# iPieter/llmq

Measured on AMD Instinct MI355X. Metric: output_tokens_per_sec (Tower-Plus-9B continuous-batching serving decode), higher is better.
Workload: dtype bf16; 1 GPU; model=tower-plus-9b (gemma-2-9b arch, random init), global_batch=512, seq_len=1024, parallelism=dp1, kv_cache_dtype=auto

## Files before the change

### llmq_amd/engine/model_runner.py

```python

from __future__ import annotations

import logging
import time
from typing import Dict, List, Optional, Tuple

import numpy as np
import torch

from llmq_amd import ops
from llmq_amd.engine.config import EngineConfig
from llmq_amd.engine.forward_meta import ChunkGather, DecodeMeta, MixedMeta, PrefillMeta
from llmq_amd.engine.kv_cache import KVCache
from llmq_amd.engine.models.llama import CausalLM
from llmq_amd.engine.scheduler import ScheduledBatch, Sequence

logger = logging.getLogger(__name__)


def _buckets(max_bs: int) -> List[int]:
    sizes = [1, 2, 4, 8, 16, 24, 32, 48, 64, 96, 128, 192, 256, 384, 512]
    out = [b for b in sizes if b < max_bs]
    out.append(max_bs)
    return out
# ... 4 lines not shown
        self,
        model: CausalLM,
        kv_cache: KVCache,
        config: EngineConfig,
        device: torch.device,
        max_model_len: int,
    ):
        self.model = model
        self.kv_cache = kv_cache
        self.config = config
        self.device = device
        self.max_model_len = max_model_len
        self.block_size = kv_cache.block_size
        self.max_blocks_per_seq = (max_model_len + self.block_size - 1) // self.block_size
        self.use_graphs = (
            config.enable_hipgraph
            and not config.enforce_eager
            and device.type == "cuda"
        )
        self._graphs: Dict[int, torch.cuda.CUDAGraph] = {}
        self._graph_pool = None
        self.sampling_generator = torch.Generator(device=device if device.type == "cuda" else "cpu")
        self.sampling_generator.manual_seed(config.seed)
        self._sample_step = 0
        self._sample_bufs: Dict[str, Dict[str, torch.Tensor]] = {}
        if self.use_graphs:
            self._alloc_static_buffers()


    def _alloc_static_buffers(self) -> None:
        B = min(self.config.max_num_seqs, self.config.hipgraph_max_batch)
        dev = self.device
        self.graph_max_bs = B
        self.in_ids = torch.zeros(B, dtype=torch.long, device=dev)
        self.in_pos = torch.zeros(B, dtype=torch.long, device=dev)
        self.in_slots = torch.zeros(B, dtype=torch.long, device=dev)
        self.in_block_tables = torch.zeros(
            B, self.max_blocks_per_seq, dtype=torch.int32, device=dev
        )
        self.in_context_lens = torch.ones(B, dtype=torch.int32, device=dev)
        self.out_hidden = torch.zeros(
            B, self.model.spec.hidden_size, dtype=self.model.dtype, device=dev
        )
        self.h_ids = torch.zeros(B, dtype=torch.long, pin_memory=True)
        self.h_pos = torch.zeros(B, dtype=torch.long, pin_memory=True)
        self.h_slots = torch.zeros(B, dtype=torch.long, pin_memory=True)
        self.h_block_tables = torch.zeros(
            B, self.max_blocks_per_seq, dtype=torch.int32, pin_memory=True
        )
        self.h_context_lens = torch.ones(B, dtype=torch.int32, pin_memory=True)
        self._staged_rows: List[Tuple[int, int, int]] = [(-1, -1, 0)] * B

    def capture_graphs(self) -> None:
        if not self.use_graphs:
            return
        t0 = time.perf_counter()
        torch.cuda.synchronize()
        for bs in reversed(_buckets(self.graph_max_bs)):
            meta = DecodeMeta(
                block_tables=self.in_block_tables[:bs],
                context_lens=self.in_context_lens[:bs],
                slot_mapping=self.in_slots[:bs],
            )
            out = self.model.forward(self.in_ids[:bs], self.in_pos[:bs], self.kv_cache, meta)
            torch.cuda.synchronize()
            graph = torch.cuda.CUDAGraph()
            with torch.cuda.graph(graph, pool=self._graph_pool):
                out = self.model.forward(
                    self.in_ids[:bs], self.in_pos[:bs], self.kv_cache, meta
                )
                self.out_hidden[:bs].copy_(out)
            if self._graph_pool is None:
                self._graph_pool = graph.pool()
            self._graphs[bs] = graph
        torch.cuda.synchronize()
        logger.info(
            "captured %d decode hipGraphs (max_bs=%d) in %.1fs",
            len(self._graphs), self.graph_max_bs, time.perf_counter() - t0,
        )

    def _bucket_for(self, bs: int) -> Optional[int]:
        for b in _buckets(self.graph_max_bs):
            if b >= bs:
                return b
        return None


    def _build_prefill_meta(self, pseqs, chunks, dev) -> tuple:
        bs = self.block_size
        ids: List[int] = []
        pos: List[int] = []
        slots: List[int] = []
        cu = [0]
        cu_k = [0]
        rel_last: List[int] = []
        any_chunk = any(start > 0 for (start, _e) in chunks)
        g_blocks: List[int] = []
        g_offs: List[int] = []
        past_dst: List[int] = []
        fresh_dst: List[int] = []
        krow = 0
        for seq, (start, end) in zip(pseqs, chunks):
            n = end - start
            ids.extend(seq.token_ids[start:end])
            pos.extend(range(start, end))
            bt = seq.block_table
            slots.extend(bt[p // bs] * bs + (p % bs) for p in range(start, end))
            if end == seq.num_tokens:
                rel_last.append(cu[-1] + n - 1)
            cu.append(cu[-1] + n)
            if any_chunk:
                for p in range(start):
                    g_blocks.append(bt[p // bs])
                    g_offs.append(p % bs)
                    past_dst.append(krow)
                    krow += 1
                for i in range(cu[-2], cu[-1]):
                    fresh_dst.append(krow)
                    krow += 1
            cu_k.append(cu_k[-1] + end)
        slot_mapping = torch.tensor(slots, dtype=torch.long, device=dev)
        gather = None
        if any_chunk:
            gather = ChunkGather(
                cu_seqlens_k=torch.tensor(cu_k, dtype=torch.int32, device=dev),
                blocks=torch.tensor(g_blocks, dtype=torch.long, device=dev),
                offs=torch.tensor(g_offs, dtype=torch.long, device=dev),
                past_dst=torch.tensor(past_dst, dtype=torch.long, device=dev),
                fresh_dst=torch.tensor(fresh_dst, dtype=torch.long, device=dev),
                total_k=krow,
            )
        meta = PrefillMeta(
            cu_seqlens=torch.tensor(cu, dtype=torch.int32, device=dev),
            max_seqlen=max(e - st for (st, e) in chunks),
            slot_mapping=slot_mapping,
            gather=gather,
        )
        return ids, pos, slot_mapping, meta, rel_last

    @torch.no_grad()
    def execute_prefill(self, seqs: List[Sequence], chunks=None, buf_name: str = "main") -> torch.Tensor:
        if chunks is None:
            chunks = [(0, s.num_tokens) for s in seqs]
        dev = self.device
        ids, pos, slot_mapping, meta, rel_last = self._build_prefill_meta(
            seqs, chunks, dev
        )
        input_ids = torch.tensor(ids, dtype=torch.long, device=dev)
        positions = torch.tensor(pos, dtype=torch.long, device=dev)
        hidden = self.model.forward(input_ids, positions, self.kv_cache, meta)
        if not rel_last:
            return torch.empty(0, dtype=torch.long, device=dev)
        last_hidden = hidden[torch.tensor(rel_last, dtype=torch.long, device=dev)]
        logits = self.model.compute_logits(last_hidden)
        sample_seqs = [s for s, (st, e) in zip(seqs, chunks) if e == s.num_tokens]
        return self._sample(logits, sample_seqs, buf_name)


    @torch.no_grad()
    def execute_mixed(self, batch: "ScheduledBatch") -> torch.Tensor:
        dev = self.device
        dseqs = batch.seqs[: batch.n_decode]
        pseqs = batch.seqs[batch.n_decode :]
        chunks = batch.chunks or [(0, s.num_tokens) for s in pseqs]
        bs = self.block_size
        nd = len(dseqs)

        ids = [s.token_ids[-1] for s in dseqs]
        pos = [s.num_tokens - 1 for s in dseqs]
        slots = [s.block_table[p // bs] * bs + (p % bs) for s, p in zip(dseqs, pos)]
        ctx = [s.num_tokens for s in dseqs]
        p_ids, p_pos, p_slots, pmeta, rel_last = self._build_prefill_meta(
            pseqs, chunks, dev
        )
        ids.extend(p_ids)
        pos.extend(p_pos)

        block_tables = torch.zeros(
            nd, max(len(s.block_table) for s in dseqs), dtype=torch.int32, device=dev
        )
        bt_np = np.zeros(tuple(block_tables.shape), dtype=np.int32)
        for i, s in enumerate(dseqs):
            bt_np[i, : len(s.block_table)] = s.block_table
        block_tables.copy_(torch.from_numpy(bt_np))
        d_slots = torch.tensor(slots, dtype=torch.long, device=dev)
        slot_mapping = torch.cat([d_slots, p_slots])
        meta = MixedMeta(
            n_decode=nd,
            decode=DecodeMeta(
                block_tables=block_tables,
                context_lens=torch.tensor(ctx, dtype=torch.int32, device=dev),
                slot_mapping=d_slots,
            ),
            prefill=pmeta,
            slot_mapping=slot_mapping,
        )
        input_ids = torch.tensor(ids, dtype=torch.long, device=dev)
        positions = torch.tensor(pos, dtype=torch.long, device=dev)
        hidden = self.model.forward(input_ids, positions, self.kv_cache, meta)
        last_idx = list(range(nd)) + [nd + r for r in rel_last]
        last_hidden = hidden[torch.tensor(last_idx, dtype=torch.long, device=dev)]
        logits = self.model.compute_logits(last_hidden)
        sample_seqs = list(dseqs) + [
            s for s, (st, e) in zip(pseqs, chunks) if e == s.num_tokens
        ]
        return self._sample(logits, sample_seqs)


    @torch.no_grad()
    def execute_decode(self, seqs: List[Sequence], force_eager: bool = False) -> torch.Tensor:
        dev = self.device
        B = len(seqs)
        bs = self.block_size
        ids = [s.token_ids[-1] for s in seqs]
        pos = [s.num_tokens - 1 for s in seqs]
        slots = [s.block_table[p // bs] * bs + (p % bs) for s, p in zip(seqs, pos)]
        ctx = [s.num_tokens for s in seqs]

        bucket = self._bucket_for(B) if (self.use_graphs and not force_eager) else None
        if bucket is not None and bucket in self._graphs:
            return self._decode_with_graph(seqs, bucket, ids, pos, slots, ctx)

        block_tables = torch.zeros(
            B, max(len(s.block_table) for s in seqs), dtype=torch.int32, device=dev
        )
        bt_np = np.zeros(tuple(block_tables.shape), dtype=np.int32)
        for i, s in enumerate(seqs):
            bt_np[i, : len(s.block_table)] = s.block_table
        block_tables.copy_(torch.from_numpy(bt_np))
        meta = DecodeMeta(
            block_tables=block_tables,
            context_lens=torch.tensor(ctx, dtype=torch.int32, device=dev),
            slot_mapping=torch.tensor(slots, dtype=torch.long, device=dev),
        )
        input_ids = torch.tensor(ids, dtype=torch.long, device=dev)
        positions = torch.tensor(pos, dtype=torch.long, device=dev)
        hidden = self.model.forward(input_ids, positions, self.kv_cache, meta)
        logits = self.model.compute_logits(hidden)
        return self._sample(logits, seqs)

    def _decode_with_graph(
        self, seqs: List[Sequence], bucket: int, ids, pos, slots, ctx
    ) -> torch.Tensor:
        B = len(seqs)
        self.h_ids[:B] = torch.tensor(ids, dtype=torch.long)
        self.h_pos[:B] = torch.tensor(pos, dtype=torch.long)
        self.h_slots[:B] = torch.tensor(slots, dtype=torch.long)
        self.h_context_lens[:B] = torch.tensor(ctx, dtype=torch.int32)
        self.h_context_lens[B:bucket] = 1
        bt_np = self.h_block_tables.numpy()
        max_w = 1
        for i, s in enumerate(seqs):
            n = len(s.block_table)
            if n > max_w:
                max_w = n
            if self._staged_rows[i] != (s.uid, s.num_preemptions, n):
                bt_np[i, :n] = s.block_table
                self._staged_rows[i] = (s.uid, s.num_preemptions, n)
        if B < bucket:
            self.h_slots[B:bucket] = 0
            self.h_ids[B:bucket] = 0
            self.h_pos[B:bucket] = 0
            for i in range(B, bucket):
                if self._staged_rows[i] != (-1, -1, 0):
                    bt_np[i, :1] = 0
                    self._staged_rows[i] = (-1, -1, 0)
        self.in_ids[:bucket].copy_(self.h_ids[:bucket], non_blocking=True)
        self.in_pos[:bucket].copy_(self.h_pos[:bucket], non_blocking=True)
        self.in_slots[:bucket].copy_(self.h_slots[:bucket], non_blocking=True)
        self.in_context_lens[:bucket].copy_(self.h_context_lens[:bucket], non_blocking=True)
        self.in_block_tables[:bucket, :max_w].copy_(
            self.h_block_tables[:bucket, :max_w], non_blocking=True
        )
        self._graphs[bucket].replay()
        logits = self.model.compute_logits(self.out_hidden[:B])
        return self._sample(logits, seqs)


    def _sample_buf(self, name: str, B: int, dev) -> Dict[str, torch.Tensor]:
        buf = self._sample_bufs.get(name)
        if buf is None or buf["out"].numel() < B:
            cap = max(B, self.config.max_num_seqs)
            buf = {
                "out": torch.empty(cap, dtype=torch.int64, device=dev),
                "keys": torch.empty(cap, dtype=torch.int64, device=dev),
                "temps": torch.empty(cap, dtype=torch.float32, device=dev),
                "temps_h": torch.empty(cap, dtype=torch.float32, pin_memory=True),
                "seeds": torch.empty(cap, dtype=torch.int32, device=dev),
                "seeds_h": torch.empty(cap, dtype=torch.int32, pin_memory=True),
                "pos": torch.empty(cap, dtype=torch.int32, device=dev),
                "pos_h": torch.empty(cap, dtype=torch.int32, pin_memory=True),
            }
            self._sample_bufs[name] = buf
        return buf

    def _sample(self, logits: torch.Tensor, seqs: List[Sequence],
                buf_name: str = "main") -> torch.Tensor:
        dev = logits.device
        self._sample_step += 1
        simple = all(
            s.params.top_k == 0 and s.params.top_p >= 1.0 for s in seqs
        )
        if dev.type == "cuda":
            B = len(seqs)
            buf = self._sample_buf(buf_name, B, dev)
            th = buf["temps_h"]
            sh = buf["seeds_h"]
            ph = buf["pos_h"]
            for i, s in enumerate(seqs):
                th[i] = s.params.temperature
                rs = s.params.seed
                if rs is None:
                    sh[i] = 0
                else:
                    v = rs & 0x7FFFFFFF
                    sh[i] = v if v else 0x1E3779B9
                ph[i] = s.output_len
            buf["temps"][:B].copy_(th[:B], non_blocking=True)
            buf["seeds"][:B].copy_(sh[:B], non_blocking=True)
            buf["pos"][:B].copy_(ph[:B], non_blocking=True)
            logits_f = logits.float()
            bounds = None
            if not simple:
                tps = torch.tensor([s.params.top_p for s in seqs],
                                   dtype=torch.float32, device=dev)
                tks = torch.tensor([s.params.top_k for s in seqs],
                                   dtype=torch.int64, device=dev)
                bounds = ops.topk_topp_bound(
                    logits_f, buf["temps"][:B], tps, tks)
            ops.sample_gumbel_argmax(
                buf["out"][:B], buf["keys"][:B], logits_f,
                buf["temps"][:B], buf["seeds"][:B],
                buf["pos"][:B], self.config.seed, self._sample_step, bounds,
            )
            return buf["out"][:B]
        temps = torch.tensor([s.params.temperature for s in seqs], dtype=torch.float32, device=dev)
        tps = torch.tensor([s.params.top_p for s in seqs], dtype=torch.float32, device=dev)
        tks = torch.tensor([s.params.top_k for s in seqs], dtype=torch.int64, device=dev)
        out = ops.sample_tokens(logits, temps, tps, tks, self.sampling_generator)
        seeded = [
            i for i, s in enumerate(seqs)
            if s.params.seed is not None and s.params.temperature > 0
        ]
        if seeded:
            idx = torch.tensor(seeded, dtype=torch.long, device=dev)
            rows = logits[idx].float().cpu()
            temps_c, tps_c, tks_c = temps[idx].cpu(), tps[idx].cpu(), tks[idx].cpu()
            redraw = torch.empty(len(seeded), dtype=out.dtype)
            for j, i in enumerate(seeded):
                s = seqs[i]
                g = torch.Generator(device="cpu")
                g.manual_seed((s.params.seed << 20) ^ s.output_len)
                redraw[j] = ops.sample_tokens(
                    rows[j : j + 1], temps_c[j : j + 1], tps_c[j : j + 1],
                    tks_c[j : j + 1], g,
                )[0]
            out[idx] = redraw.to(out.device)
        return out
```

### llmq_amd/engine/models/llama.py

```python

from __future__ import annotations

import math
import os
from typing import Dict, List, Optional, Union

import torch
import torch.nn.functional as F

from llmq_amd import ops
from llmq_amd.engine.forward_meta import DecodeMeta, MixedMeta, PrefillMeta
from llmq_amd.engine.kv_cache import KVCache
from llmq_amd.engine.model_specs import ModelSpec
from llmq_amd.parallel import get_tp_group


_USE_SKINNY_GEMM = os.environ.get("LLMQ_SKINNY_GEMM", "0") not in ("0", "false", "")


def _proj(x: torch.Tensor, w: torch.Tensor, bias=None) -> torch.Tensor:
    if (_USE_SKINNY_GEMM and x.is_cuda and x.dtype == torch.bfloat16
            and x.shape[0] <= 1024 and w.shape[1] % 64 == 0
            and w.shape[0] % 4 == 0):
        return ops.skinny_gemm(x, w, bias)
# ... 104 lines not shown
        h = self.spec.hidden_size
        std = 0.02
        out_std = std / math.sqrt(2 * self.spec.num_layers)
        fill(self.embedding, std)
        for lw in self.layers:
            lw.input_norm.fill_(1.0 - self.norm_offset)
            fill(lw.qkv, std)
            if lw.qkv_bias is not None:
                lw.qkv_bias.zero_()
            fill(lw.o, out_std)
            lw.pre_mlp_norm.fill_(1.0 - self.norm_offset)
            fill(lw.gate_up, std)
            fill(lw.down, out_std)
            if lw.post_attn_norm is not None:
                lw.post_attn_norm.fill_(1.0 - self.norm_offset)
                lw.post_mlp_norm.fill_(1.0 - self.norm_offset)
        self.final_norm.fill_(1.0 - self.norm_offset)
        if not self.spec.tied_embeddings:
            fill(self.lm_head, std)

    def named_tensors(self) -> Dict[str, torch.Tensor]:
        out = {"embedding": self.embedding, "final_norm": self.final_norm}
        if not self.spec.tied_embeddings:
            out["lm_head"] = self.lm_head
        for i, lw in enumerate(self.layers):
            p = f"layers.{i}."
            out[p + "input_norm"] = lw.input_norm
            out[p + "qkv"] = lw.qkv
            if lw.qkv_bias is not None:
                out[p + "qkv_bias"] = lw.qkv_bias
            out[p + "o"] = lw.o
            out[p + "pre_mlp_norm"] = lw.pre_mlp_norm
            out[p + "gate_up"] = lw.gate_up
            out[p + "down"] = lw.down
            if lw.post_attn_norm is not None:
                out[p + "post_attn_norm"] = lw.post_attn_norm
                out[p + "post_mlp_norm"] = lw.post_mlp_norm
        return out

    def weight_bytes(self) -> int:
        return sum(t.numel() * t.element_size() for t in self.named_tensors().values())


    def _norm(self, x: torch.Tensor, w: torch.Tensor) -> torch.Tensor:
        return ops.rmsnorm(x, w, self.spec.rms_eps, self.norm_offset)

    def _prefill_attn(self, q, k, v, pmeta, kv_cache, layer: int, window: int):
        s = self.spec
        g = pmeta.gather
        if g is None:
            return ops.varlen_prefill_attention(
                q, k, v, pmeta.cu_seqlens, pmeta.max_seqlen, s.scale,
                s.attn_softcap, window,
            )
        KVH, D = k.shape[1], k.shape[2]
        k_att = q.new_empty(g.total_k, KVH, D)
        v_att = q.new_empty(g.total_k, KVH, D)
        past_k = kv_cache.k[layer][g.blocks, :, g.offs].to(q.dtype)
        past_v = kv_cache.v[layer][g.blocks, :, g.offs].to(q.dtype)
        k_att.index_copy_(0, g.past_dst, past_k)
        v_att.index_copy_(0, g.past_dst, past_v)
        k_att.index_copy_(0, g.fresh_dst, k)
        v_att.index_copy_(0, g.fresh_dst, v)
        return ops.varlen_prefill_attention(
            q, k_att, v_att, pmeta.cu_seqlens, pmeta.max_seqlen, s.scale,
            s.attn_softcap, window, cu_seqlens_k=g.cu_seqlens_k,
        )

    @torch.no_grad()
    def forward(
        self,
        input_ids: torch.Tensor,
        positions: torch.Tensor,
        kv_cache: KVCache,
        meta: Union[PrefillMeta, DecodeMeta, MixedMeta],
    ) -> torch.Tensor:
        s = self.spec
        tp = get_tp_group() if self.tp_size > 1 else None
        x = F.embedding(input_ids, self.embedding)
        if s.embedding_scale:
            x = x * math.sqrt(s.hidden_size)
            x = x.to(self.dtype)
        residual = x
        h = self._norm(x, self.layers[0].input_norm)
        n_layers = len(self.layers)
        for i, lw in enumerate(self.layers):
            qkv = _proj(h, lw.qkv, lw.qkv_bias)
            q, k, v = qkv.split([self.q_size, self.kv_size, self.kv_size], dim=-1)
            T = q.shape[0]
            q = q.view(T, self.heads, s.head_dim)
            k = k.view(T, self.kv_heads, s.head_dim)
            v = v.view(T, self.kv_heads, s.head_dim)
            ops.rope_and_cache(
                q, k, v, kv_cache.k[i], kv_cache.v[i], positions,
                self.rope_cache, meta.slot_mapping,
            )
            window = s.sliding_window if s.layer_uses_sliding_window(i) else 0
            if meta.is_prefill:
                attn = self._prefill_attn(q, k, v, meta, kv_cache, i, window)
            elif meta.is_mixed:
                nd = meta.n_decode
                attn_d = ops.paged_decode_attention(
                    q[:nd], kv_cache.k[i], kv_cache.v[i],
                    meta.decode.block_tables, meta.decode.context_lens,
                    s.scale, s.attn_softcap, window,
                )
                attn_p = self._prefill_attn(
                    q[nd:], k[nd:], v[nd:], meta.prefill, kv_cache, i, window
                )
                attn = torch.cat([attn_d, attn_p], dim=0)
            else:
                attn = ops.paged_decode_attention(
                    q, kv_cache.k[i], kv_cache.v[i], meta.block_tables,
                    meta.context_lens, s.scale, s.attn_softcap, window,
                )
            attn_out = _proj(attn.reshape(T, self.q_size), lw.o)
            if tp is not None:
                attn_out = tp.all_reduce(attn_out)
            if s.post_norms:
                h, residual = ops.norm_add_norm(
                    attn_out, residual, lw.post_attn_norm, lw.pre_mlp_norm,
                    s.rms_eps, self.norm_offset,
                )
            else:
                h, residual = ops.fused_add_rmsnorm(
                    attn_out, residual, lw.pre_mlp_norm, s.rms_eps, self.norm_offset
                )
            gate_up = _proj(h, lw.gate_up)
            act = ops.gelu_tanh_and_mul(gate_up) if s.gelu else ops.silu_and_mul(gate_up)
            mlp_out = _proj(act, lw.down)
            if tp is not None:
                mlp_out = tp.all_reduce(mlp_out)
            w_next = (
                self.layers[i + 1].input_norm if i + 1 < n_layers else self.final_norm
            )
            if s.post_norms:
                h, residual = ops.norm_add_norm(
                    mlp_out, residual, lw.post_mlp_norm, w_next,
                    s.rms_eps, self.norm_offset,
                )
            else:
                h, residual = ops.fused_add_rmsnorm(
                    mlp_out, residual, w_next, s.rms_eps, self.norm_offset
                )
        return h

    @torch.no_grad()
    def compute_logits(self, hidden: torch.Tensor) -> torch.Tensor:
        logits = _proj(hidden, self.lm_head).float()
        cap = self.spec.final_softcap
        if cap and cap > 0:
            logits = torch.tanh(logits / cap) * cap
        return logits
```

### llmq_amd/ops/__init__.py

```python

from __future__ import annotations

import os
from pathlib import Path
from typing import Optional, Tuple

import torch

from llmq_amd.ops import torch_ref

_EXT = None
_EXT_ERROR: Optional[str] = None
_EXT_TRIED = False


def _try_load_extension() -> None:
    global _EXT, _EXT_ERROR, _EXT_TRIED
    if _EXT_TRIED:
        return
    _EXT_TRIED = True
    here = Path(__file__).parent
    override = os.environ.get("LLMQ_OPS_SO")
    if override:
        candidates = [Path(override)]
# ... 54 lines not shown


def norm_add_norm(
    x: torch.Tensor, residual: torch.Tensor, w_post: torch.Tensor,
    w_pre: torch.Tensor, eps: float, offset: float = 0.0,
) -> Tuple[torch.Tensor, torch.Tensor]:
    if _use_hip(x):
        _EXT.norm_add_norm(x, residual, w_post, w_pre, eps, offset)
        return x, residual
    return torch_ref.norm_add_norm(x, residual, w_post, w_pre, eps, offset)




def rope_inplace(
    q: torch.Tensor, k: torch.Tensor, positions: torch.Tensor, cos_sin: torch.Tensor
) -> None:
    if _use_hip(q):
        _EXT.rope_inplace(q, k, positions, cos_sin)
        return
    torch_ref.rope_inplace(q, k, positions, cos_sin)


build_rope_cache = torch_ref.build_rope_cache




def silu_and_mul(x: torch.Tensor) -> torch.Tensor:
    if _use_hip(x):
        d = x.shape[-1] // 2
        out = torch.empty(*x.shape[:-1], d, dtype=x.dtype, device=x.device)
        _EXT.silu_and_mul(out, x)
        return out
    return torch_ref.silu_and_mul(x)


def gelu_tanh_and_mul(x: torch.Tensor) -> torch.Tensor:
    if _use_hip(x):
        d = x.shape[-1] // 2
        out = torch.empty(*x.shape[:-1], d, dtype=x.dtype, device=x.device)
        _EXT.gelu_tanh_and_mul(out, x)
        return out
    return torch_ref.gelu_tanh_and_mul(x)


def rope_and_cache(
    q: torch.Tensor, k: torch.Tensor, v: torch.Tensor,
    k_cache: torch.Tensor, v_cache: torch.Tensor,
    positions: torch.Tensor, cos_sin: torch.Tensor, slot_mapping: torch.Tensor,
) -> None:
    if _use_hip(q):
        _EXT.rope_and_cache(q, k, v, k_cache, v_cache, positions, cos_sin, slot_mapping)
        return
    torch_ref.rope_inplace(q, k, positions, cos_sin)
    torch_ref.reshape_and_cache(k, v, k_cache, v_cache, slot_mapping)




def reshape_and_cache(
    key: torch.Tensor,
    value: torch.Tensor,
    k_cache: torch.Tensor,
    v_cache: torch.Tensor,
    slot_mapping: torch.Tensor,
) -> None:
    if _use_hip(key):
        _EXT.reshape_and_cache(key, value, k_cache, v_cache, slot_mapping)
        return
    torch_ref.reshape_and_cache(key, value, k_cache, v_cache, slot_mapping)




def paged_decode_attention(
    q: torch.Tensor,
    k_cache: torch.Tensor,
    v_cache: torch.Tensor,
    block_tables: torch.Tensor,
    context_lens: torch.Tensor,
    scale: float,
    softcap: float = 0.0,
    window: int = 0,
) -> torch.Tensor:
    if _use_hip(q):
        out = torch.empty_like(q)
        _EXT.paged_decode_attention(
            out, q, k_cache, v_cache, block_tables, context_lens, scale, softcap, window
        )
        return out
    return torch_ref.paged_decode_attention(
        q, k_cache, v_cache, block_tables, context_lens, scale, softcap, window
    )


def varlen_prefill_attention(
    q: torch.Tensor,
    k: torch.Tensor,
    v: torch.Tensor,
    cu_seqlens: torch.Tensor,
    max_seqlen: int,
    scale: float,
    softcap: float = 0.0,
    window: int = 0,
    cu_seqlens_k: Optional[torch.Tensor] = None,
) -> torch.Tensor:
    cu_k = cu_seqlens if cu_seqlens_k is None else cu_seqlens_k
    if _use_hip(q):
        out = torch.empty_like(q)
        _EXT.varlen_prefill_attention(
            out, q, k, v, cu_seqlens, cu_k, int(max_seqlen), scale, softcap, window
        )
        return out
    return torch_ref.varlen_prefill_attention(
        q, k, v, cu_seqlens, scale, softcap, window, cu_seqlens_k=cu_k
    )




def skinny_gemm(
    x: torch.Tensor,
    w: torch.Tensor,
    bias: Optional[torch.Tensor] = None,
    splitk: int = 0,
    out: Optional[torch.Tensor] = None,
) -> torch.Tensor:
    M, K = x.shape
    N = w.shape[0]
    if not (x.is_cuda and x.dtype == torch.bfloat16 and K % 64 == 0
            and N % 4 == 0 and has_hip_ext()):
        import torch.nn.functional as F

        return F.linear(x, w, bias)
    if out is None:
        out = torch.empty(M, N, dtype=torch.bfloat16, device=x.device)
    _EXT.skinny_gemm(out, x, w, bias, splitk)
    return out




def sample_gumbel_argmax(
    out: torch.Tensor,
    keys: torch.Tensor,
    logits: torch.Tensor,
    temps: torch.Tensor,
    req_seeds: torch.Tensor,
    req_pos: torch.Tensor,
    seed: int,
    step: int,
    bounds: Optional[torch.Tensor] = None,
) -> None:
    assert _use_hip(logits)
    keys.zero_()
    _EXT.sample_gumbel_argmax(out, keys, logits, temps, req_seeds, req_pos,
                              seed, step, bounds)


def topk_topp_bound(
    logits: torch.Tensor,
    temps: torch.Tensor,
    top_ps: torch.Tensor,
    top_ks: torch.Tensor,
) -> torch.Tensor:
    assert _use_hip(logits)
    out = torch.empty(logits.size(0), dtype=torch.float32, device=logits.device)
    _EXT.topk_topp_bound(out, logits, temps, top_ps, top_ks)
    return out


def sample_tokens(
    logits: torch.Tensor,
    temperatures: torch.Tensor,
    top_ps: torch.Tensor,
    top_ks: torch.Tensor,
    generator: Optional[torch.Generator] = None,
) -> torch.Tensor:
    if logits.is_cuda:
        return _sample_tokens_gpu(logits, temperatures, top_ps, top_ks, generator)
    return torch_ref.sample_tokens(logits, temperatures, top_ps, top_ks, generator)


def _sample_tokens_gpu(
    logits: torch.Tensor,
    temperatures: torch.Tensor,
    top_ps: torch.Tensor,
    top_ks: torch.Tensor,
    generator: Optional[torch.Generator],
) -> torch.Tensor:
    B, V = logits.shape
    greedy = temperatures <= 0
    temps = torch.where(greedy, torch.ones_like(temperatures), temperatures)
    scaled = logits.float() / temps.unsqueeze(1)
    need_topk = bool((top_ks > 0).any()) and bool((top_ks < V).any())
    need_topp = bool((top_ps < 1.0).any())
    if need_topk or need_topp:
        bound = topk_topp_bound(logits.float(), temperatures.float(),
                                top_ps.float(), top_ks)
        scaled = torch.where(logits.float() >= bound.unsqueeze(1), scaled,
                             torch.full_like(scaled, float("-inf")))
    u = torch.rand(B, V, device=logits.device, generator=generator)
    gumbel = -torch.log(-torch.log(u.clamp_min(1e-20)).clamp_min(1e-20))
    sampled = (scaled + gumbel).argmax(dim=-1)
    greedy_choice = logits.argmax(dim=-1)
    return torch.where(greedy, greedy_choice, sampled)
```

### llmq_amd/ops/hip/bindings.cpp

```cpp

#include <ATen/ATen.h>
#include <c10/hip/HIPStream.h>
#include <hip/hip_runtime.h>
#include <torch/library.h>

#include <hip/hip_bf16.h>
#include <hip/hip_fp16.h>


namespace {

#define CHECK_GPU(x) TORCH_CHECK(x.is_cuda(), #x " must be on GPU")
#define CHECK_LASTDIM(x) \
  TORCH_CHECK(x.stride(-1) == 1, #x " innermost dim must be contiguous")

hipStream_t stream() { return c10::hip::getCurrentHIPStream().stream(); }

template <typename F>
void dispatch_dtype(const at::Tensor& t, const char* name, F&& f) {
  switch (t.scalar_type()) {
    case at::kBFloat16:
      f.template operator()<__hip_bfloat16>();
      break;
    case at::kHalf:
// ... 350 lines not shown

void paged_decode_attention(at::Tensor out, at::Tensor q, at::Tensor k_cache,
                            at::Tensor v_cache, at::Tensor block_tables,
                            at::Tensor context_lens, double scale,
                            double softcap, long window) {
  CHECK_GPU(q);
  CHECK_LASTDIM(q);
  TORCH_CHECK(block_tables.scalar_type() == at::kInt);
  TORCH_CHECK(context_lens.scalar_type() == at::kInt);
  dispatch_dtype(q, "paged_decode_attention", [&]<typename T>() {
    launch_decode<T>(out, q, k_cache, v_cache, block_tables, context_lens,
                     scale, softcap, window);
  });
}

template <typename T>
void launch_prefill(at::Tensor& out, const at::Tensor& q, const at::Tensor& k,
                    const at::Tensor& v, const at::Tensor& cu,
                    const at::Tensor& cu_k, int B,
                    double scale, double softcap, long window, long max_seqlen) {
  const int H = q.size(1), D = q.size(2);
  const int KVH = k.size(1);
  if constexpr (std::is_same_v<T, __hip_bfloat16>) {
    const int qtiles = (int)((max_seqlen + 63) / 64);
    dim3 fgrid(B, H, std::max(qtiles, 1));
    const char* ppe = getenv("LLMQ_PREFILL_PIPE");
    const bool use_pipe = !ppe || atoi(ppe) != 0;
    auto lf = [&]<int HD>() {
      if (use_pipe) {
        hipLaunchKernelGGL((flash_prefill_pipe_kernel<HD>), fgrid, dim3(256), 0,
                           stream(),
                           reinterpret_cast<__hip_bfloat16*>(out.data_ptr()),
                           reinterpret_cast<const __hip_bfloat16*>(q.data_ptr()),
                           reinterpret_cast<const __hip_bfloat16*>(k.data_ptr()),
                           reinterpret_cast<const __hip_bfloat16*>(v.data_ptr()),
                           cu.data_ptr<int>(), cu_k.data_ptr<int>(), H, KVH,
                           (float)scale, (float)softcap, (int)window,
                           q.stride(0), k.stride(0), v.stride(0), out.stride(0));
        return;
      }
      hipLaunchKernelGGL((flash_prefill_bf16_kernel<HD>), fgrid, dim3(256), 0,
                         stream(),
                         reinterpret_cast<__hip_bfloat16*>(out.data_ptr()),
                         reinterpret_cast<const __hip_bfloat16*>(q.data_ptr()),
                         reinterpret_cast<const __hip_bfloat16*>(k.data_ptr()),
                         reinterpret_cast<const __hip_bfloat16*>(v.data_ptr()),
                         cu.data_ptr<int>(), cu_k.data_ptr<int>(), H, KVH,
                         (float)scale, (float)softcap, (int)window,
                         q.stride(0), k.stride(0), v.stride(0), out.stride(0));
    };
    switch (D) {
      case 64: lf.template operator()<64>(); return;
      case 128: lf.template operator()<128>(); return;
      case 256: lf.template operator()<256>(); return;
      default: TORCH_CHECK(false, "unsupported head_dim ", D);
    }
  }
  dim3 grid(B, H);
  auto l = [&]<int HD>() {
    hipLaunchKernelGGL((varlen_prefill_attention_kernel<T, HD>), grid,
                       dim3(256), 0, stream(),
                       reinterpret_cast<T*>(out.data_ptr()),
                       reinterpret_cast<const T*>(q.data_ptr()),
                       reinterpret_cast<const T*>(k.data_ptr()),
                       reinterpret_cast<const T*>(v.data_ptr()),
                       cu.data_ptr<int>(), cu_k.data_ptr<int>(), H, KVH,
                       (float)scale, (float)softcap, (int)window,
                       q.stride(0), k.stride(0), v.stride(0), out.stride(0));
  };
  switch (D) {
    case 64: l.template operator()<64>(); break;
    case 128: l.template operator()<128>(); break;
    case 256: l.template operator()<256>(); break;
    default: TORCH_CHECK(false, "unsupported head_dim ", D);
  }
}

void varlen_prefill_attention(at::Tensor out, at::Tensor q, at::Tensor k,
                              at::Tensor v, at::Tensor cu_seqlens,
                              at::Tensor cu_seqlens_k,
                              long max_seqlen, double scale, double softcap,
                              long window) {
  CHECK_GPU(q);
  CHECK_LASTDIM(q);
  TORCH_CHECK(cu_seqlens.scalar_type() == at::kInt);
  TORCH_CHECK(cu_seqlens_k.scalar_type() == at::kInt);
  const int B = cu_seqlens.size(0) - 1;
  dispatch_dtype(q, "varlen_prefill_attention", [&]<typename T>() {
    launch_prefill<T>(out, q, k, v, cu_seqlens, cu_seqlens_k, B, scale,
                      softcap, window, max_seqlen);
  });
}


void skinny_gemm(at::Tensor out, at::Tensor x, at::Tensor w,
                 c10::optional<at::Tensor> bias, long splitk) {
  CHECK_GPU(x);
  CHECK_LASTDIM(x);
  CHECK_LASTDIM(w);
  TORCH_CHECK(x.scalar_type() == at::kBFloat16 && w.scalar_type() == at::kBFloat16);
  TORCH_CHECK(out.scalar_type() == at::kBFloat16 && out.is_contiguous());
  const int M = x.size(0), K = x.size(1), N = w.size(0);
  TORCH_CHECK(w.size(1) == K && out.size(0) == M && out.size(1) == N);
  TORCH_CHECK(K % SKG_BK == 0, "K must be a multiple of 64");
  TORCH_CHECK(N % 4 == 0, "N must be a multiple of 4");
  const __hip_bfloat16* bias_ptr = nullptr;
  if (bias.has_value() && bias->defined()) {
    TORCH_CHECK(bias->scalar_type() == at::kBFloat16 && bias->numel() == N);
    bias_ptr = reinterpret_cast<const __hip_bfloat16*>(bias->data_ptr());
  }
  const int mt = (M + SKG_BM - 1) / SKG_BM;
  const int nt = (N + SKG_BN - 1) / SKG_BN;
  int z = (int)splitk;
  if (z <= 0) {
    z = 1;
    while (mt * nt * z < 256 && (K / SKG_BK) / (z * 2) >= 8 && z < 8) z *= 2;
  }
  dim3 grid(mt, nt, z);
  static const int sync_dbg = [] {
    const char* e = getenv("LLMQ_SKG_SYNC");
    return e ? atoi(e) : 0;
  }();
  if (z == 1) {
    if (sync_dbg) {
      hipLaunchKernelGGL((skinny_gemm_kernel<0, 1>), grid, dim3(SKG_NT), 0,
                         stream(), out.data_ptr(),
                         reinterpret_cast<const __hip_bfloat16*>(x.data_ptr()),
                         reinterpret_cast<const __hip_bfloat16*>(w.data_ptr()),
                         bias_ptr, M, N, K, x.stride(0), w.stride(0));
      return;
    }
    hipLaunchKernelGGL((skinny_gemm_kernel<0>), grid, dim3(SKG_NT), 0, stream(),
                       out.data_ptr(),
                       reinterpret_cast<const __hip_bfloat16*>(x.data_ptr()),
                       reinterpret_cast<const __hip_bfloat16*>(w.data_ptr()),
                       bias_ptr, M, N, K, x.stride(0), w.stride(0));
    return;
  }
  at::Tensor slabs = at::empty({z, (long)M * N}, x.options().dtype(at::kFloat));
  hipLaunchKernelGGL((skinny_gemm_kernel<1>), grid, dim3(SKG_NT), 0, stream(),
                     slabs.data_ptr(),
                     reinterpret_cast<const __hip_bfloat16*>(x.data_ptr()),
                     reinterpret_cast<const __hip_bfloat16*>(w.data_ptr()),
                     nullptr, M, N, K, x.stride(0), w.stride(0));
  const long MN = (long)M * N;
  const long blocks = (MN / 4 + 255) / 256;
  hipLaunchKernelGGL(skinny_gemm_reduce_kernel, dim3(blocks), dim3(256), 0,
                     stream(),
                     reinterpret_cast<__hip_bfloat16*>(out.data_ptr()),
                     slabs.data_ptr<float>(), bias_ptr, z, MN, N);
}


void topk_topp_bound(at::Tensor out_bound, at::Tensor logits, at::Tensor temps,
                     at::Tensor top_ps, at::Tensor top_ks) {
  CHECK_GPU(logits);
  TORCH_CHECK(logits.scalar_type() == at::kFloat && logits.dim() == 2);
  TORCH_CHECK(out_bound.scalar_type() == at::kFloat);
  TORCH_CHECK(top_ps.scalar_type() == at::kFloat);
  TORCH_CHECK(top_ks.scalar_type() == at::kLong);
  const int B = logits.size(0), V = logits.size(1);
  hipLaunchKernelGGL(topk_topp_bound_kernel, dim3(B), dim3(256), 0, stream(),
                     out_bound.data_ptr<float>(), logits.data_ptr<float>(),
                     temps.data_ptr<float>(), top_ps.data_ptr<float>(),
                     top_ks.data_ptr<long>(), V, logits.stride(0));
}

void sample_gumbel_argmax(at::Tensor out, at::Tensor keys, at::Tensor logits,
                          at::Tensor temps, at::Tensor req_seeds,
                          at::Tensor req_pos, long seed, long step,
                          c10::optional<at::Tensor> bounds) {
  CHECK_GPU(logits);
  TORCH_CHECK(logits.scalar_type() == at::kFloat && logits.dim() == 2);
  TORCH_CHECK(out.scalar_type() == at::kLong);
  TORCH_CHECK(keys.scalar_type() == at::kLong && keys.numel() == logits.size(0));
  TORCH_CHECK(req_seeds.scalar_type() == at::kInt);
  TORCH_CHECK(req_pos.scalar_type() == at::kInt);
  const int B = logits.size(0), V = logits.size(1);
  const float* bounds_ptr = nullptr;
  if (bounds.has_value() && bounds->defined()) {
    TORCH_CHECK(bounds->scalar_type() == at::kFloat && bounds->numel() == B);
    bounds_ptr = bounds->data_ptr<float>();
  }
  int nsplit = 1;
  while (B * nsplit < 2048 && nsplit < 64 && (V / nsplit) > 4096) nsplit *= 2;
  hipLaunchKernelGGL(sample_argmax_kernel, dim3(B, nsplit), dim3(256), 0,
                     stream(),
                     reinterpret_cast<unsigned long long*>(keys.data_ptr()),
                     logits.data_ptr<float>(), temps.data_ptr<float>(),
                     reinterpret_cast<const unsigned int*>(req_seeds.data_ptr()),
                     reinterpret_cast<const unsigned int*>(req_pos.data_ptr()),
                     bounds_ptr, V, (unsigned int)seed, (unsigned int)step);
  hipLaunchKernelGGL(unpack_keys_kernel, dim3((B + 255) / 256), dim3(256), 0,
                     stream(), out.data_ptr<long>(),
                     reinterpret_cast<const unsigned long long*>(keys.data_ptr()),
                     B);
}

}

TORCH_LIBRARY(llmq_amd, m) {
  m.def("rmsnorm(Tensor(a!) out, Tensor input, Tensor weight, float eps, float offset) -> ()");
  m.def("fused_add_rmsnorm(Tensor(a!) x, Tensor(b!) residual, Tensor weight, float eps, float offset) -> ()");
  m.def("silu_and_mul(Tensor(a!) out, Tensor input) -> ()");
  m.def("gelu_tanh_and_mul(Tensor(a!) out, Tensor input) -> ()");
  m.def("rope_inplace(Tensor(a!) q, Tensor(b!) k, Tensor positions, Tensor cos_sin) -> ()");
  m.def("reshape_and_cache(Tensor key, Tensor value, Tensor(a!) k_cache, Tensor(b!) v_cache, Tensor slot_mapping) -> ()");
  m.def("paged_decode_attention(Tensor(a!) out, Tensor q, Tensor k_cache, Tensor v_cache, Tensor block_tables, Tensor context_lens, float scale, float softcap, int window) -> ()");
  m.def("varlen_prefill_attention(Tensor(a!) out, Tensor q, Tensor k, Tensor v, Tensor cu_seqlens, Tensor cu_seqlens_k, int max_seqlen, float scale, float softcap, int window) -> ()");
  m.def("sample_gumbel_argmax(Tensor(a!) out, Tensor(b!) keys, Tensor logits, Tensor temps, Tensor req_seeds, Tensor req_pos, int seed, int step, Tensor? bounds=None) -> ()");
  m.def("topk_topp_bound(Tensor(a!) out_bound, Tensor logits, Tensor temps, Tensor top_ps, Tensor top_ks) -> ()");
  m.def("skinny_gemm(Tensor(a!) out, Tensor x, Tensor w, Tensor? bias, int splitk) -> ()");
  m.def("norm_add_norm(Tensor(a!) x, Tensor(b!) residual, Tensor w_post, Tensor w_pre, float eps, float offset) -> ()");
  m.def("rope_and_cache(Tensor(a!) q, Tensor(b!) k, Tensor value, Tensor(c!) k_cache, Tensor(d!) v_cache, Tensor positions, Tensor cos_sin, Tensor slot_mapping) -> ()");
}

TORCH_LIBRARY_IMPL(llmq_amd, CUDA, m) {
  m.impl("rmsnorm", &rmsnorm);
  m.impl("fused_add_rmsnorm", &fused_add_rmsnorm);
  m.impl("silu_and_mul", &silu_and_mul);
  m.impl("gelu_tanh_and_mul", &gelu_tanh_and_mul);
  m.impl("rope_inplace", &rope_inplace);
  m.impl("reshape_and_cache", &reshape_and_cache);
  m.impl("paged_decode_attention", &paged_decode_attention);
  m.impl("varlen_prefill_attention", &varlen_prefill_attention);
  m.impl("sample_gumbel_argmax", &sample_gumbel_argmax);
  m.impl("topk_topp_bound", &topk_topp_bound);
  m.impl("skinny_gemm", &skinny_gemm);
  m.impl("norm_add_norm", &norm_add_norm);
  m.impl("rope_and_cache", &rope_and_cache);
}
```

### llmq_amd/ops/hip/sampling.hip

```cpp

#include "common.h"

DEVINL unsigned int hash_u32(unsigned int x) {
  x ^= x >> 16; x *= 0x7feb352dU;
  x ^= x >> 15; x *= 0x846ca68bU;
  x ^= x >> 16;
  return x;
}

DEVINL float uniform01(unsigned int seed, unsigned int step, unsigned int b,
                       unsigned int v) {
  unsigned int key = b * 0x9E3779B9u ^ v * 0x85EBCA6Bu ^ step * 0xC2B2AE35u ^ seed;
  unsigned int h = hash_u32(hash_u32(key));
  return (h + 1u) * (1.0f / 4294967296.0f);
}

DEVINL unsigned long long pack_key(float val, int idx) {
  unsigned int u = __float_as_uint(val);
  u = (u & 0x80000000u) ? ~u : (u | 0x80000000u);
  return ((unsigned long long)u << 32) | (unsigned int)(~idx);
}

__global__ __launch_bounds__(256) void sample_argmax_kernel(
    unsigned long long* __restrict__ out_keys,
    const float* __restrict__ logits,
    const float* __restrict__ temps,
    const unsigned int* __restrict__ req_seeds,
    const unsigned int* __restrict__ req_pos,
    const float* __restrict__ bounds,
    int V, unsigned int seed, unsigned int step) {
  const int b = blockIdx.x;
  const int nsplit = gridDim.y;
  const int chunk = (V + nsplit - 1) / nsplit;
  const int v0 = blockIdx.y * chunk;
  const int v1 = min(v0 + chunk, V);
  const float temp = temps[b];
  const bool greedy = temp <= 0.f;
  const float inv_t = greedy ? 1.0f : 1.0f / temp;
  const float* row = logits + (long)b * V;
  const unsigned int rs = req_seeds[b];
  const unsigned int kseed = rs ? rs : seed;
  const unsigned int kstep = rs ? req_pos[b] : step;
  const unsigned int kb = rs ? 0u : (unsigned int)b;
  const float bound = bounds ? bounds[b] : -3e38f;

  float best = -3e38f;
  int best_i = v0;
  for (int v = v0 + threadIdx.x; v < v1; v += 256) {
    if (row[v] < bound) continue;
    float x = row[v] * inv_t;
    if (!greedy) {
      const float u = uniform01(kseed, kstep, kb, v);
      x += -__logf(-__logf(u));
    }
    if (x > best) { best = x; best_i = v; }
  }
  for (int off = WAVE / 2; off > 0; off >>= 1) {
    const float ov = __shfl_xor(best, off, WAVE);
    const int oi = __shfl_xor(best_i, off, WAVE);
    if (ov > best || (ov == best && oi < best_i)) { best = ov; best_i = oi; }
  }
  __shared__ float vals[4];
  __shared__ int idxs[4];
  const int wid = threadIdx.x / WAVE;
  if ((threadIdx.x & (WAVE - 1)) == 0) { vals[wid] = best; idxs[wid] = best_i; }
  __syncthreads();
  if (threadIdx.x == 0) {
    for (int w = 1; w < 4; ++w) {
      if (vals[w] > best || (vals[w] == best && idxs[w] < best_i)) {
        best = vals[w]; best_i = idxs[w];
      }
    }
    atomicMax(out_keys + b, pack_key(best, best_i));
  }
}


#define TH_NBINS 512
#define TH_TPB 256
#define TH_XMIN -32.0f

__global__ __launch_bounds__(TH_TPB) void topk_topp_bound_kernel(
    float* __restrict__ out_bound,
    const float* __restrict__ logits,
    const float* __restrict__ temps,
    const float* __restrict__ top_ps,
    const long* __restrict__ top_ks,
    int V, long stride) {
  const int b = blockIdx.x;
  const int tid = threadIdx.x;
  const float T0 = temps[b];
  const float p_lim = top_ps[b];
  const long k_lim = top_ks[b];
  const bool need_p = p_lim < 1.0f;
  const bool need_k = k_lim > 0 && k_lim < V;
  if (T0 <= 0.f || !(need_p || need_k)) {
    if (tid == 0) out_bound[b] = -3e38f;
    return;
  }
  const float inv_t = 1.0f / T0;
  const float* row = logits + (long)b * stride;

  __shared__ float h_sum[TH_NBINS];
  __shared__ int h_cnt[TH_NBINS];
  __shared__ float red[TH_TPB / WAVE];
  __shared__ float sh_state[6];

  float m = -3e38f;
  for (int v = tid; v < V; v += TH_TPB) m = fmaxf(m, row[v]);
  for (int off = WAVE / 2; off > 0; off >>= 1)
    m = fmaxf(m, __shfl_xor(m, off, WAVE));
  if ((tid & (WAVE - 1)) == 0) red[tid / WAVE] = m;
  __syncthreads();
  if (tid == 0) {
    for (int w = 1; w < TH_TPB / WAVE; ++w) m = fmaxf(m, red[w]);
    red[0] = m;
  }
  __syncthreads();
  m = red[0];

  float xlo = TH_XMIN, xhi = 0.0f;
  float keep_above = 3e38f;
  float p_above = 0.f;
  long n_above = 0;
  float Z = 0.f;
  float bound_x = TH_XMIN;
  bool done = false;

  for (int iter = 0; iter < 2 && !done; ++iter) {
    for (int i = tid; i < TH_NBINS; i += TH_TPB) { h_sum[i] = 0.f; h_cnt[i] = 0; }
    __syncthreads();
    const float w = (xhi - xlo) / TH_NBINS;
    const float inv_w = 1.0f / w;
    float tail = 0.f;
    for (int v = tid; v < V; v += TH_TPB) {
      const float x = (row[v] - m) * inv_t;
      if (x >= keep_above) continue;
      if (x < xlo) { if (iter == 0) tail += __expf(fmaxf(x, -80.f)); continue; }
      int bin = (int)((x - xlo) * inv_w);
      bin = bin < 0 ? 0 : (bin >= TH_NBINS ? TH_NBINS - 1 : bin);
      atomicAdd(&h_sum[bin], __expf(x));
      atomicAdd(&h_cnt[bin], 1);
    }
    for (int off = WAVE / 2; off > 0; off >>= 1) tail += __shfl_xor(tail, off, WAVE);
    if ((tid & (WAVE - 1)) == 0) red[tid / WAVE] = tail;
    __syncthreads();
    if (tid == 0) {
      if (iter == 0) {
        Z = red[0] + red[1] + red[2] + red[3];
        for (int i = 0; i < TH_NBINS; ++i) Z += h_sum[i];
        sh_state[3] = Z;
      } else {
        Z = sh_state[3];
      }
      const float p_target = need_p ? p_lim * Z : 3e38f;
      const long k_target = need_k ? k_lim : 0x7fffffffffffffffL;
      float cum = p_above;
      long cnt = n_above;
      int cross = -1;
      for (int i = TH_NBINS - 1; i >= 0; --i) {
        cum += h_sum[i];
        cnt += h_cnt[i];
        if (cum >= p_target || cnt >= k_target) { cross = i; break; }
      }
      if (cross < 0) {
        sh_state[0] = (iter == 0) ? -3e38f : xlo;
        sh_state[1] = 1.0f;
      } else {
        float pa = p_above;
        long na = n_above;
        for (int i = TH_NBINS - 1; i > cross; --i) { pa += h_sum[i]; na += h_cnt[i]; }
        sh_state[0] = xlo + cross * w;
        sh_state[1] = 0.0f;
        sh_state[2] = xlo + (cross + 1) * w;
        sh_state[4] = (cross == TH_NBINS - 1) ? keep_above
                                              : (xlo + (cross + 1) * w);
        red[0] = pa;
        red[1] = (float)na;
      }
    }
    __syncthreads();
    if (sh_state[1] != 0.0f) {
      bound_x = sh_state[0];
      done = true;
    } else {
      xlo = sh_state[0];
      xhi = sh_state[2];
      keep_above = sh_state[4];
      p_above = red[0];
      n_above = (long)red[1];
      bound_x = xlo;
    }
    __syncthreads();
  }
  if (tid == 0)
    out_bound[b] = (bound_x <= -3e37f) ? -3e38f : (m + bound_x * T0);
}

__global__ void unpack_keys_kernel(long* __restrict__ out,
                                   const unsigned long long* __restrict__ keys,
                                   int B) {
  const int b = blockIdx.x * blockDim.x + threadIdx.x;
  if (b < B) out[b] = (long)(unsigned int)(~(keys[b] & 0xffffffffu));
}
```

Measured before the change: 10500 tokens/s.

## Fuse final logit softcap and bf16 read into sampling kernels

Logits now come straight from the LM-head projection in bf16 without the separate tanh softcap pass and without a float32 conversion. The sampling and top-k/top-p kernels are templated on element type, apply the softcap inline on load, and read bf16 with 16-byte vector loads. This removes several elementwise passes and an fp32 copy over the large vocab logits matrix each decode step. In exchange the sampling kernels do tanh per element, and the top-p path computes it repeatedly across its passes.

New measurement: 10600 tokens/s (median of 6 runs). Within noise of the previous version (+1.0%).

```diff
diff --git a/llmq_amd/engine/model_runner.py b/llmq_amd/engine/model_runner.py
--- a/llmq_amd/engine/model_runner.py
+++ b/llmq_amd/engine/model_runner.py
@@ -180,9 +180,9 @@
         if not rel_last:
             return torch.empty(0, dtype=torch.long, device=dev)
         last_hidden = hidden[torch.tensor(rel_last, dtype=torch.long, device=dev)]
-        logits = self.model.compute_logits(last_hidden)
+        logits, cap = self._logits(last_hidden)
         sample_seqs = [s for s, (st, e) in zip(seqs, chunks) if e == s.num_tokens]
-        return self._sample(logits, sample_seqs, buf_name)
+        return self._sample(logits, sample_seqs, buf_name, softcap=cap)
 
 
     @torch.no_grad()
@@ -228,11 +228,11 @@
         hidden = self.model.forward(input_ids, positions, self.kv_cache, meta)
         last_idx = list(range(nd)) + [nd + r for r in rel_last]
         last_hidden = hidden[torch.tensor(last_idx, dtype=torch.long, device=dev)]
-        logits = self.model.compute_logits(last_hidden)
+        logits, cap = self._logits(last_hidden)
         sample_seqs = list(dseqs) + [
             s for s, (st, e) in zip(pseqs, chunks) if e == s.num_tokens
         ]
-        return self._sample(logits, sample_seqs)
+        return self._sample(logits, sample_seqs, softcap=cap)
 
 
     @torch.no_grad()
@@ -264,8 +264,8 @@
         input_ids = torch.tensor(ids, dtype=torch.long, device=dev)
         positions = torch.tensor(pos, dtype=torch.long, device=dev)
         hidden = self.model.forward(input_ids, positions, self.kv_cache, meta)
-        logits = self.model.compute_logits(hidden)
-        return self._sample(logits, seqs)
+        logits, cap = self._logits(hidden)
+        return self._sample(logits, seqs, softcap=cap)
 
     def _decode_with_graph(
         self, seqs: List[Sequence], bucket: int, ids, pos, slots, ctx
@@ -301,8 +301,8 @@
             self.h_block_tables[:bucket, :max_w], non_blocking=True
         )
         self._graphs[bucket].replay()
-        logits = self.model.compute_logits(self.out_hidden[:B])
-        return self._sample(logits, seqs)
+        logits, cap = self._logits(self.out_hidden[:B])
+        return self._sample(logits, seqs, softcap=cap)
 
 
     def _sample_buf(self, name: str, B: int, dev) -> Dict[str, torch.Tensor]:
@@ -322,8 +322,13 @@
             self._sample_bufs[name] = buf
         return buf
 
+    def _logits(self, hidden: torch.Tensor):
+        if hidden.device.type == "cuda":
+            return self.model.compute_logits_raw(hidden)
+        return self.model.compute_logits(hidden), 0.0
+
     def _sample(self, logits: torch.Tensor, seqs: List[Sequence],
-                buf_name: str = "main") -> torch.Tensor:
+                buf_name: str = "main", softcap: float = 0.0) -> torch.Tensor:
         dev = logits.device
         self._sample_step += 1
         simple = all(
@@ -347,7 +352,6 @@
             buf["temps"][:B].copy_(th[:B], non_blocking=True)
             buf["seeds"][:B].copy_(sh[:B], non_blocking=True)
             buf["pos"][:B].copy_(ph[:B], non_blocking=True)
-            logits_f = logits.float()
             bounds = None
             if not simple:
                 tps = torch.tensor([s.params.top_p for s in seqs],
@@ -355,11 +359,12 @@
                 tks = torch.tensor([s.params.top_k for s in seqs],
                                    dtype=torch.int64, device=dev)
                 bounds = ops.topk_topp_bound(
-                    logits_f, buf["temps"][:B], tps, tks)
+                    logits, buf["temps"][:B], tps, tks, softcap)
             ops.sample_gumbel_argmax(
-                buf["out"][:B], buf["keys"][:B], logits_f,
+                buf["out"][:B], buf["keys"][:B], logits,
                 buf["temps"][:B], buf["seeds"][:B],
                 buf["pos"][:B], self.config.seed, self._sample_step, bounds,
+                softcap,
             )
             return buf["out"][:B]
         temps = torch.tensor([s.params.temperature for s in seqs], dtype=torch.float32, device=dev)
diff --git a/llmq_amd/engine/models/llama.py b/llmq_amd/engine/models/llama.py
--- a/llmq_amd/engine/models/llama.py
+++ b/llmq_amd/engine/models/llama.py
@@ -280,3 +280,8 @@
         if cap and cap > 0:
             logits = torch.tanh(logits / cap) * cap
         return logits
+
+    @torch.no_grad()
+    def compute_logits_raw(self, hidden: torch.Tensor):
+        cap = self.spec.final_softcap
+        return _proj(hidden, self.lm_head), float(cap) if cap and cap > 0 else 0.0
diff --git a/llmq_amd/ops/__init__.py b/llmq_amd/ops/__init__.py
--- a/llmq_amd/ops/__init__.py
+++ b/llmq_amd/ops/__init__.py
@@ -230,11 +230,12 @@
     seed: int,
     step: int,
     bounds: Optional[torch.Tensor] = None,
+    softcap: float = 0.0,
 ) -> None:
     assert _use_hip(logits)
     keys.zero_()
     _EXT.sample_gumbel_argmax(out, keys, logits, temps, req_seeds, req_pos,
-                              seed, step, bounds)
+                              seed, step, bounds, float(softcap))
 
 
 def topk_topp_bound(
@@ -242,10 +243,11 @@
     temps: torch.Tensor,
     top_ps: torch.Tensor,
     top_ks: torch.Tensor,
+    softcap: float = 0.0,
 ) -> torch.Tensor:
     assert _use_hip(logits)
     out = torch.empty(logits.size(0), dtype=torch.float32, device=logits.device)
-    _EXT.topk_topp_bound(out, logits, temps, top_ps, top_ks)
+    _EXT.topk_topp_bound(out, logits, temps, top_ps, top_ks, float(softcap))
     return out
 
 
diff --git a/llmq_amd/ops/hip/bindings.cpp b/llmq_amd/ops/hip/bindings.cpp
--- a/llmq_amd/ops/hip/bindings.cpp
+++ b/llmq_amd/ops/hip/bindings.cpp
@@ -526,31 +526,52 @@
 }
 
 
+static float host_inv_cap(double softcap) {
+  const float cap = (float)softcap;
+  return cap > 0.f ? 1.0f / cap : 0.f;
+}
+static void check_logits(const at::Tensor& logits) {
+  CHECK_GPU(logits);
+  TORCH_CHECK(logits.dim() == 2 && logits.stride(1) == 1,
+              "logits must be [B, V] with unit element stride");
+  TORCH_CHECK(logits.scalar_type() == at::kFloat ||
+                  logits.scalar_type() == at::kBFloat16,
+              "logits must be fp32 or bf16");
+}
+
 void topk_topp_bound(at::Tensor out_bound, at::Tensor logits, at::Tensor temps,
-                     at::Tensor top_ps, at::Tensor top_ks) {
-  CHECK_GPU(logits);
-  TORCH_CHECK(logits.scalar_type() == at::kFloat && logits.dim() == 2);
+                     at::Tensor top_ps, at::Tensor top_ks, double softcap) {
+  check_logits(logits);
   TORCH_CHECK(out_bound.scalar_type() == at::kFloat);
   TORCH_CHECK(top_ps.scalar_type() == at::kFloat);
   TORCH_CHECK(top_ks.scalar_type() == at::kLong);
   const int B = logits.size(0), V = logits.size(1);
-  hipLaunchKernelGGL(topk_topp_bound_kernel, dim3(B), dim3(256), 0, stream(),
-                     out_bound.data_ptr<float>(), logits.data_ptr<float>(),
-                     temps.data_ptr<float>(), top_ps.data_ptr<float>(),
-                     top_ks.data_ptr<long>(), V, logits.stride(0));
+  if (B == 0 || V == 0) return;
+  auto launch = [&](auto* lp) {
+    using T = std::remove_cv_t<std::remove_pointer_t<decltype(lp)>>;
+    hipLaunchKernelGGL((topk_topp_bound_kernel<T>), dim3(B), dim3(256), 0,
+                       stream(), out_bound.data_ptr<float>(), lp,
+                       temps.data_ptr<float>(), top_ps.data_ptr<float>(),
+                       top_ks.data_ptr<long>(), V, (long)logits.stride(0),
+                       (float)softcap, host_inv_cap(softcap));
+  };
+  if (logits.scalar_type() == at::kFloat)
+    launch(logits.data_ptr<float>());
+  else
+    launch(reinterpret_cast<const __hip_bfloat16*>(logits.data_ptr()));
 }
 
 void sample_gumbel_argmax(at::Tensor out, at::Tensor keys, at::Tensor logits,
                           at::Tensor temps, at::Tensor req_seeds,
                           at::Tensor req_pos, long seed, long step,
-                          c10::optional<at::Tensor> bounds) {
-  CHECK_GPU(logits);
-  TORCH_CHECK(logits.scalar_type() == at::kFloat && logits.dim() == 2);
+                          c10::optional<at::Tensor> bounds, double softcap) {
+  check_logits(logits);
   TORCH_CHECK(out.scalar_type() == at::kLong);
   TORCH_CHECK(keys.scalar_type() == at::kLong && keys.numel() == logits.size(0));
   TORCH_CHECK(req_seeds.scalar_type() == at::kInt);
   TORCH_CHECK(req_pos.scalar_type() == at::kInt);
   const int B = logits.size(0), V = logits.size(1);
+  if (B == 0) return;
   const float* bounds_ptr = nullptr;
   if (bounds.has_value() && bounds->defined()) {
     TORCH_CHECK(bounds->scalar_type() == at::kFloat && bounds->numel() == B);
@@ -558,13 +579,21 @@
   }
   int nsplit = 1;
   while (B * nsplit < 2048 && nsplit < 64 && (V / nsplit) > 4096) nsplit *= 2;
-  hipLaunchKernelGGL(sample_argmax_kernel, dim3(B, nsplit), dim3(256), 0,
-                     stream(),
-                     reinterpret_cast<unsigned long long*>(keys.data_ptr()),
-                     logits.data_ptr<float>(), temps.data_ptr<float>(),
-                     reinterpret_cast<const unsigned int*>(req_seeds.data_ptr()),
-                     reinterpret_cast<const unsigned int*>(req_pos.data_ptr()),
-                     bounds_ptr, V, (unsigned int)seed, (unsigned int)step);
+  auto launch = [&](auto* lp) {
+    using T = std::remove_cv_t<std::remove_pointer_t<decltype(lp)>>;
+    hipLaunchKernelGGL(
+        (sample_argmax_kernel<T>), dim3(B, nsplit), dim3(256), 0, stream(),
+        reinterpret_cast<unsigned long long*>(keys.data_ptr()), lp,
+        temps.data_ptr<float>(),
+        reinterpret_cast<const unsigned int*>(req_seeds.data_ptr()),
+        reinterpret_cast<const unsigned int*>(req_pos.data_ptr()), bounds_ptr,
+        V, (long)logits.stride(0), (float)softcap, host_inv_cap(softcap),
+        (unsigned int)seed, (unsigned int)step);
+  };
+  if (logits.scalar_type() == at::kFloat)
+    launch(static_cast<const float*>(logits.data_ptr<float>()));
+  else
+    launch(reinterpret_cast<const __hip_bfloat16*>(logits.data_ptr()));
   hipLaunchKernelGGL(unpack_keys_kernel, dim3((B + 255) / 256), dim3(256), 0,
                      stream(), out.data_ptr<long>(),
                      reinterpret_cast<const unsigned long long*>(keys.data_ptr()),
@@ -582,8 +611,8 @@
   m.def("reshape_and_cache(Tensor key, Tensor value, Tensor(a!) k_cache, Tensor(b!) v_cache, Tensor slot_mapping) -> ()");
   m.def("paged_decode_attention(Tensor(a!) out, Tensor q, Tensor k_cache, Tensor v_cache, Tensor block_tables, Tensor context_lens, float scale, float softcap, int window) -> ()");
   m.def("varlen_prefill_attention(Tensor(a!) out, Tensor q, Tensor k, Tensor v, Tensor cu_seqlens, Tensor cu_seqlens_k, int max_seqlen, float scale, float softcap, int window) -> ()");
-  m.def("sample_gumbel_argmax(Tensor(a!) out, Tensor(b!) keys, Tensor logits, Tensor temps, Tensor req_seeds, Tensor req_pos, int seed, int step, Tensor? bounds=None) -> ()");
-  m.def("topk_topp_bound(Tensor(a!) out_bound, Tensor logits, Tensor temps, Tensor top_ps, Tensor top_ks) -> ()");
+  m.def("sample_gumbel_argmax(Tensor(a!) out, Tensor(b!) keys, Tensor logits, Tensor temps, Tensor req_seeds, Tensor req_pos, int seed, int step, Tensor? bounds=None, float softcap=0.0) -> ()");
+  m.def("topk_topp_bound(Tensor(a!) out_bound, Tensor logits, Tensor temps, Tensor top_ps, Tensor top_ks, float softcap=0.0) -> ()");
   m.def("skinny_gemm(Tensor(a!) out, Tensor x, Tensor w, Tensor? bias, int splitk) -> ()");
   m.def("norm_add_norm(Tensor(a!) x, Tensor(b!) residual, Tensor w_post, Tensor w_pre, float eps, float offset) -> ()");
   m.def("rope_and_cache(Tensor(a!) q, Tensor(b!) k, Tensor value, Tensor(c!) k_cache, Tensor(d!) v_cache, Tensor positions, Tensor cos_sin, Tensor slot_mapping) -> ()");
diff --git a/llmq_amd/ops/hip/sampling.hip b/llmq_amd/ops/hip/sampling.hip
--- a/llmq_amd/ops/hip/sampling.hip
+++ b/llmq_amd/ops/hip/sampling.hip
@@ -21,40 +21,76 @@
   return ((unsigned long long)u << 32) | (unsigned int)(~idx);
 }
 
+DEVINL float softcap_exact(float x, float cap, float inv_cap) {
+  return tanhf(x * inv_cap) * cap;
+}
+
+template <typename T>
+DEVINL float load_logit(const T* p, bool capped, float cap, float inv_cap) {
+  const float x = to_f32(*p);
+  return capped ? softcap_exact(x, cap, inv_cap) : x;
+}
+
+template <typename T>
 __global__ __launch_bounds__(256) void sample_argmax_kernel(
     unsigned long long* __restrict__ out_keys,
-    const float* __restrict__ logits,
+    const T* __restrict__ logits,
     const float* __restrict__ temps,
     const unsigned int* __restrict__ req_seeds,
     const unsigned int* __restrict__ req_pos,
     const float* __restrict__ bounds,
-    int V, unsigned int seed, unsigned int step) {
+    int V, long stride, float softcap, float inv_cap, unsigned int seed,
+    unsigned int step) {
+  constexpr int VE = Vec8<T>::kElems;
   const int b = blockIdx.x;
   const int nsplit = gridDim.y;
   const int chunk = (V + nsplit - 1) / nsplit;
-  const int v0 = blockIdx.y * chunk;
+  const int v0 = min((int)blockIdx.y * chunk, V);
   const int v1 = min(v0 + chunk, V);
   const float temp = temps[b];
   const bool greedy = temp <= 0.f;
   const float inv_t = greedy ? 1.0f : 1.0f / temp;
-  const float* row = logits + (long)b * V;
+  const T* row = logits + (long)b * stride;
   const unsigned int rs = req_seeds[b];
   const unsigned int kseed = rs ? rs : seed;
   const unsigned int kstep = rs ? req_pos[b] : step;
   const unsigned int kb = rs ? 0u : (unsigned int)b;
   const float bound = bounds ? bounds[b] : -3e38f;
+  const bool capped = softcap > 0.f;
 
   float best = -3e38f;
   int best_i = v0;
-  for (int v = v0 + threadIdx.x; v < v1; v += 256) {
-    if (row[v] < bound) continue;
-    float x = row[v] * inv_t;
+  auto consider = [&](float l, int v) {
+    if (l < bound) return;
+    float x = l * inv_t;
     if (!greedy) {
       const float u = uniform01(kseed, kstep, kb, v);
       x += -__logf(-__logf(u));
     }
     if (x > best) { best = x; best_i = v; }
-  }
+  };
+
+  const unsigned long addr0 = (unsigned long)(row + v0);
+  const int mis = (int)((addr0 & 15u) / sizeof(T));
+  const int va = min(v0 + ((VE - mis) & (VE - 1)), v1);
+  const int nvec = (v1 - va) / VE;
+  const int vb = va + nvec * VE;
+
+  for (int v = v0 + threadIdx.x; v < va; v += 256)
+    consider(load_logit(row + v, capped, softcap, inv_cap), v);
+  for (int i = threadIdx.x; i < nvec; i += 256) {
+    const int v = va + i * VE;
+    const Vec8<T> pk = load16(row + v);
+#pragma unroll
+    for (int j = 0; j < VE; ++j) {
+      float l = to_f32(pk.data[j]);
+      if (capped) l = softcap_exact(l, softcap, inv_cap);
+      consider(l, v + j);
+    }
+  }
+  for (int v = vb + threadIdx.x; v < v1; v += 256)
+    consider(load_logit(row + v, capped, softcap, inv_cap), v);
+
   for (int off = WAVE / 2; off > 0; off >>= 1) {
     const float ov = __shfl_xor(best, off, WAVE);
     const int oi = __shfl_xor(best_i, off, WAVE);
@@ -80,15 +116,17 @@
 #define TH_TPB 256
 #define TH_XMIN -32.0f
 
+template <typename T>
 __global__ __launch_bounds__(TH_TPB) void topk_topp_bound_kernel(
     float* __restrict__ out_bound,
-    const float* __restrict__ logits,
+    const T* __restrict__ logits,
     const float* __restrict__ temps,
     const float* __restrict__ top_ps,
     const long* __restrict__ top_ks,
-    int V, long stride) {
+    int V, long stride, float softcap, float inv_cap) {
   const int b = blockIdx.x;
   const int tid = threadIdx.x;
+  const bool capped = softcap > 0.f;
   const float T0 = temps[b];
   const float p_lim = top_ps[b];
   const long k_lim = top_ks[b];
@@ -99,7 +137,7 @@
     return;
   }
   const float inv_t = 1.0f / T0;
-  const float* row = logits + (long)b * stride;
+  const T* row = logits + (long)b * stride;
 
   __shared__ float h_sum[TH_NBINS];
   __shared__ int h_cnt[TH_NBINS];
@@ -107,7 +145,7 @@
   __shared__ float sh_state[6];
 
   float m = -3e38f;
-  for (int v = tid; v < V; v += TH_TPB) m = fmaxf(m, row[v]);
+  for (int v = tid; v < V; v += TH_TPB) m = fmaxf(m, load_logit(row + v, capped, softcap, inv_cap));
   for (int off = WAVE / 2; off > 0; off >>= 1)
     m = fmaxf(m, __shfl_xor(m, off, WAVE));
   if ((tid & (WAVE - 1)) == 0) red[tid / WAVE] = m;
@@ -134,7 +172,7 @@
     const float inv_w = 1.0f / w;
     float tail = 0.f;
     for (int v = tid; v < V; v += TH_TPB) {
-      const float x = (row[v] - m) * inv_t;
+      const float x = (load_logit(row + v, capped, softcap, inv_cap) - m) * inv_t;
       if (x >= keep_above) continue;
       if (x < xlo) { if (iter == 0) tail += __expf(fmaxf(x, -80.f)); continue; }
       int bin = (int)((x - xlo) * inv_w);
```
